# populationgenomics/cuKING

Measured on AMD Instinct MI355X. Metric: sample-pairs/s (all-pairs KING), higher is better.
Workload: dtype fp4 products, f32 accumulate (exact integers)

## Files before the change

cuking_amd/csrc/king_abi.hip:

```cpp
#include <hip/hip_runtime.h>

#include <algorithm>
#include <cstdio>
#include <cstdlib>
#include <cstring>
#include <vector>

#include "king_common.h"
#include "king_geno.h"
#include "king_host.h"
#include "king_ibd.h"
#include "king_kin_summary.h"
#include "king_ld.h"
#include "king_site_qc.h"
#include "king_unrelated.h"

using namespace cuking;

namespace {

#define HIP_TRY(expr)                                                      \
  do {                                                                     \
    const hipError_t _e = (expr);                                          \
    if (_e != hipSuccess) {                                                \
// ... 380 lines not shown
  a.result_index = out.result_index;
  a.result_overflow = out.result_overflow;
  a.dense_counts = out.counts;
  a.dense_kin = out.kin;
  a.kin_ld = out.kin_ld;
  a.kin_diag = (out.kin != nullptr && (out.kin_flags & CUKING_KIN_SYMMETRIC)) ? 1u : 0u;
  a.sum_hist = reinterpret_cast<unsigned long long *>(out.sum_hist);
  a.sum_best = reinterpret_cast<unsigned long long *>(out.sum_best);
  if (out.sum_hist != nullptr) {
    a.sum_lo = out.sum_bins.lo;
    a.sum_scale = kin_bin_scale(out.sum_bins);
    a.sum_bins = out.sum_bins.num_bins;
  }
  a.rel_counts = out.rel_counts;
  if (out.rel_counts != nullptr) {
    a.rel_num = out.rel_num;
    for (uint32_t t = 0; t < out.rel_num; ++t) a.rel_thr[t] = out.rel_thr[t];
  }
  a.rect_row_stride = 1;
  a.bits = d_bit_sets;
  a.words_per_sample = words_per_sample;
  a.split_wgs = ctx->split_wgs;
  if (plan_variant(ctx, words_per_sample).layout == kLayoutNibbleStats) {
    a.perm = plane_perm(ctx->planes, geo);
    if (!ctx->prepared.codes) a.codes_ready = plane_flags(ctx->planes, geo);
  }
  cuking_ctx::StreamScratch *e;
  const cuking_status st = scratch_for(ctx, stream, block_tiles, &e);
  if (st != CUKING_OK || e == nullptr) return st;
  if (uses_split_slab(ctx)) {
    a.split_counters = e->split;
    a.split_scratch = e->split + mfma_split_counter_bytes(ctx->split_wgs) / sizeof(uint32_t);
  }
  if (!uses_filter_scratch(ctx)) return CUKING_OK;
  uint8_t *base = e->filter;
  const FilterScratchLayout l = filter_scratch_layout(e->filter_tiles);
  a.sample_stats = plane_stats(ctx->planes, geo);
  a.t2 = plane_t2(ctx->planes, geo);
  a.prefix_u = plane_prefix_u(ctx->planes, geo);
  a.cohort_sums = plane_cohort_sums(ctx->planes, geo);
  a.filter_ctrl = reinterpret_cast<uint32_t *>(base);
  a.filter_totals = reinterpret_cast<unsigned long long *>(base + l.totals);
  a.fsplit_tickets = reinterpret_cast<uint32_t *>(base + l.tickets);
  a.tile_done = base + l.tile_done;
  a.cand_list = reinterpret_cast<uint2 *>(base + l.cand);
  a.cand_cap = ctx->filter_cand_cap < l.cand_entries ? ctx->filter_cand_cap : l.cand_entries;
  a.quadrant_cap = ctx->filter_quadrant_cap;
  a.dense_list = reinterpret_cast<uint2 *>(base + l.dense);
  a.dense_cap = l.chunk_tiles * 4;
  a.fsplit_slabs = ctx->split_wgs != 0 ? reinterpret_cast<float4 *>(base + l.slabs) : nullptr;
  a.rotate_min_steps = ctx->filter_rotate_min_steps;
  a.check_steps = plane_check_steps(ctx->planes, geo);
  if (ctx->prepared.site_order) a.site_curve = plane_site_curve(ctx->planes, geo);
  a.site_rotate = ctx->filter_site_order == 2;
  return CUKING_OK;
}

hipError_t launch_planned(const cuking_ctx *ctx, uint32_t words_per_sample, bool full,
                          TiledArgs a, const LaunchSwitches &sw, uint64_t num_tiles,
                          hipStream_t stream) {
  const int kv = effective_variant(ctx, words_per_sample);
  if (tiled_variant(kv).tile != tiled_variant(ctx->variant).tile) {
    if (tiled_variant(kv).tile * 2 != tiled_variant(ctx->variant).tile) return hipErrorInvalidValue;
    to_quadrants(&a, &num_tiles);
  }
  return launch_tiled(kv, full, a, sw, num_tiles, stream);
}

void note_reader(cuking_ctx *ctx, hipStream_t stream) {
  for (auto &r : ctx->readers)
    if (r.first == stream) return;
  ctx->readers.emplace_back(stream, nullptr);
}

cuking_status wait_for_readers(cuking_ctx *ctx, hipStream_t stream) {
  bool failed = false;
  for (auto &r : ctx->readers) {
    if (r.first == stream) continue;
    if (r.second == nullptr &&
        hipEventCreateWithFlags(&r.second, hipEventDisableTiming) != hipSuccess) {
      failed = true;
      break;
    }
    if (hipEventRecord(r.second, r.first) != hipSuccess ||
        hipStreamWaitEvent(stream, r.second, 0) != hipSuccess) {
      failed = true;
      break;
    }
  }
  if (failed) {
    (void)hipGetLastError();
    ++ctx->host_syncs;
    HIP_TRY(hipDeviceSynchronize());
  }
  for (auto &r : ctx->readers)
    if (r.second) (void)hipEventDestroy(r.second);
  ctx->readers.clear();
  ctx->readers.emplace_back(stream, nullptr);
  ctx->prepared.ordered_on = stream;
  ctx->prepared.ordered_valid = true;
  for (auto &t : ctx->prepared.tiles)
    if (t == 2) t = 1;
  return CUKING_OK;
}

void mark_read(cuking_ctx *ctx, uint32_t begin, uint32_t end) {
  std::vector<uint8_t> &t = ctx->prepared.tiles;
// ... 1693 lines not shown
```

cuking_amd/csrc/king_common.h:

```cpp
#ifndef CUKING_AMD_KING_COMMON_H_
#define CUKING_AMD_KING_COMMON_H_

#include <hip/hip_runtime.h>
#include <stdint.h>

#include "cuking_amd.h"
#include "king_launch_plan.h"
#include "king_submatrix.h"

namespace cuking {

constexpr uint32_t kLayoutWord = 0;
constexpr uint32_t kLayoutQuad = 1;
constexpr uint32_t kLayoutNibble = 2;
constexpr uint32_t kLayoutNibbleStats = 3;

struct PlaneGeometry {
  uint32_t num_rows, num_cols;
  uint32_t rows_padded, cols_padded;
  uint32_t col_base;
  uint32_t s_stride;
  uint32_t k_words;
  uint32_t diag;
};
// ... 50 lines not shown
  uint32_t i_begin, j_begin;
  float kin_threshold;
  uint32_t max_results;
  cuking_result *results;
  uint32_t *result_index;
  uint32_t *result_overflow;
  cuking_counts *dense_counts;
  const uint64_t *bits;
  uint32_t words_per_sample;
  uint32_t split_tiles, split_wgs;
  uint32_t split_whole;
  uint32_t *split_scratch, *split_counters;
  uint32_t xcd_chunk, launch_tiles;
  uint32_t dyn_tiles, dyn_wgs;
  uint32_t quad;
  const uint2 *tile_list;
  const uint32_t *tile_list_count;
  uint32_t tile_list_cap;
  const float2 *sample_stats;
  const uint4 *t2;
  uint32_t *filter_ctrl;
  unsigned long long *filter_totals;
  uint2 *cand_list;
  uint32_t cand_cap;
  uint32_t quadrant_cap;
  uint2 *dense_list;
  uint32_t dense_cap;
  uint32_t fsplit_parts, fsplit_first, fsplit_tile0;
  float4 *fsplit_slabs;
  uint32_t *fsplit_tickets;
  const uint32_t *check_steps;
  const float *prefix_u;
  const unsigned long long *cohort_sums;
  uint32_t check0, check1;
  uint32_t rotate, rotate_min_steps;
  uint32_t rotate_min_tiles;
  uint8_t *tile_done;
  const uint32_t *gate;
  uint32_t gate_count;
  const uint8_t *skip_tiles;
  uint64_t skip_base;
  const uint32_t *perm;
  uint32_t *codes_ready;
  float *dense_kin;
  uint64_t kin_ld;
  uint32_t kin_diag;
  unsigned long long *sum_hist, *sum_best;
  float sum_lo, sum_scale;
  uint32_t sum_bins;
  uint32_t *rel_counts;
  uint32_t rel_num;
  float rel_thr[CUKING_REL_THRESHOLDS_MAX];
  const struct SiteCurve *site_curve;
  uint32_t site_rotate;
};

constexpr uint32_t kCheckEmitCap = 64;
constexpr uint32_t kNumCheckShares = 8;
constexpr uint32_t kCheckShares64[kNumCheckShares] = {8, 50, 53, 56, 58, 60, 61, 62};
constexpr uint32_t kNumPhases = 128;
constexpr uint32_t kPhasesPerShare = kNumPhases / 64;
constexpr uint32_t kNumCum = kNumPhases - 1;
__host__ __device__ inline uint32_t phase_step(uint32_t all_steps, uint32_t x) {
  return (uint32_t)((uint64_t)all_steps * x / kNumPhases);
}
constexpr uint64_t kSiteOrderMinTiles = 24576;
constexpr uint32_t kSiteOrderMinGain = 2;
constexpr uint32_t kSiteOrderNoTrust = 15;
struct SiteCurve {
  unsigned long long cum[kNumPhases];
  unsigned long long het_calls, missing_calls;
  float sigma;
  uint32_t pad[11];
};
static_assert(sizeof(SiteCurve) % 64 == 0, "whole 64-byte lines");
__host__ __device__ inline float site_curve_mass(const unsigned long long *cum, uint32_t phase,
                                                 uint32_t share64) {
  const uint32_t hi = phase + share64 * kPhasesPerShare;
  auto front = [&](uint32_t x) { return x == 0 ? 0ull : cum[x - 1]; };
  const unsigned long long all = cum[kNumPhases - 1];
  const unsigned long long got = hi <= kNumPhases ? front(hi) - front(phase)
                                                  : (all - front(phase)) + front(hi - kNumPhases);
  return all != 0 ? (float)got / (float)all : 0.f;
}
__host__ __device__ inline bool site_curve_covers(const unsigned long long *cum, uint32_t phase,
                                                  uint32_t share64, float need) {
  return site_curve_mass(cum, phase, share64) >= need;
}
__host__ __device__ inline uint32_t check_step_of(uint32_t all_steps, uint32_t k,
                                                  uint32_t min_steps = 64) {
  if (all_steps < min_steps) return 0;
  return phase_step(all_steps, kCheckShares64[k] * kPhasesPerShare);
}
constexpr uint32_t kFilterSplitSlabs = 256;
constexpr size_t kFilterSlabBytes = 256 * 256 * sizeof(float);
constexpr size_t kFilterTicketBytes = kFilterSplitSlabs * sizeof(uint32_t);
__host__ __device__ inline size_t plane_bytes(const PlaneGeometry &g,
                                              uint32_t layout) {
  const size_t base = (size_t)g.k_words * g.s_stride * (layout == kLayoutQuad ? 8 : 16);
  if (layout == kLayoutNibble) return base + base / 4;
  if (layout == kLayoutNibbleStats)
    return base + base / 4 + base / 2 + (size_t)g.s_stride * sizeof(float2) +
           (size_t)g.s_stride * kNumCum * sizeof(float) + 64 + 64 +
           64 + (size_t)g.s_stride * (4 + 8 + 4 * (kNumCum + 1) + 16) +
           sizeof(SiteCurve);
  return base;
}
__host__ __device__ inline const uint4 *plane_t2(const uint4 *planes, const PlaneGeometry &g) {
  return planes + (size_t)g.k_words * g.s_stride * 5 / 4;
}
__host__ __device__ inline const float2 *plane_stats(const uint4 *planes, const PlaneGeometry &g) {
  return reinterpret_cast<const float2 *>(planes + (size_t)g.k_words * g.s_stride * 7 / 4);
}
__host__ __device__ inline const float *plane_prefix_u(const uint4 *planes, const PlaneGeometry &g) {
  return reinterpret_cast<const float *>(plane_stats(planes, g) + g.s_stride);
}
__host__ __device__ inline const unsigned long long *plane_cohort_sums(const uint4 *planes,
                                                                       const PlaneGeometry &g) {
  return reinterpret_cast<const unsigned long long *>(plane_prefix_u(planes, g) +
                                                      (size_t)g.s_stride * kNumCum);
}
// ... 266 lines not shown
```

cuking_amd/csrc/king_filter.hip:

```cpp
#include <hip/hip_runtime.h>
#include <stdio.h>

#include <atomic>
#include <stdlib.h>

#include "king_common.h"
#include "king_device.h"
#include "king_kin_summary.h"

#pragma clang diagnostic ignored "-Winline-asm"

namespace cuking {

namespace {

typedef int v8i __attribute__((ext_vector_type(8)));
typedef float v16f __attribute__((ext_vector_type(16)));

constexpr int kT = (int)kFilterTile;
constexpr int kUnits = 2;
constexpr int kStages = 5;
constexpr int kSliceU4 = kT;
constexpr int kStageU4 = 2 * 2 * kUnits * kSliceU4;
constexpr int kStageReqs = 4 * kUnits;
// ... 110 lines not shown
  r[1] = (int)(w.y & mask);
  r[2] = (int)(w.z & mask);
  r[3] = (int)(w.w & mask);
  return r;
}

struct Tile {
  bool split;
  uint32_t bid;
  uint32_t tr, tc;
  uint32_t part, piece;
};

__device__ __forceinline__ bool bound_level(const unsigned long long *cohort_sums, float sites,
                                            float *mean, float *sigma) {
  const float ns = (float)cohort_sums[0], nm = (float)cohort_sums[1], nh = (float)cohort_sums[2];
  if (!(ns > 0.f && nh > 0.f)) return false;
  const float m = nm / (ns * sites), h = nh / (ns * sites);
  *mean = m * (1.f + m / (2.f * h * (1.f - m)));
  *sigma = rsqrtf(sites);
  return true;
}

__device__ __forceinline__ bool take_tile(const TiledArgs &a, const uint32_t wg, uint4 *const lds,
                                          Tile *t) {
  uint32_t bid = wg;
  t->split = a.fsplit_parts != 0 && wg >= a.fsplit_first;
  t->part = t->piece = 0;
  if (t->split) {
    t->piece = wg - a.fsplit_first;
    t->part = __builtin_amdgcn_readfirstlane(t->piece % a.fsplit_parts);
    bid = a.fsplit_tile0 + t->piece / a.fsplit_parts;
  } else
  if (a.dyn_tiles != 0 && wg >= a.launch_tiles) {
    uint32_t *slot = reinterpret_cast<uint32_t *>(lds);
    if (threadIdx.x == 0) *slot = relaxed_add(a.filter_ctrl + kCtrlDyn, 1u);
    __syncthreads();
    const uint32_t next = __builtin_amdgcn_readfirstlane(*slot);
    __syncthreads();
    if (next >= a.dyn_tiles) return false;
    bid = a.launch_tiles + next;
  } else if (a.xcd_chunk == 1) {
    bid = xcd_patch_tile(bid);
    if (bid >= a.launch_tiles) return false;
  }
  t->bid = __builtin_amdgcn_readfirstlane(bid);
  uint32_t tr, tc;
  if (!decode_tile_space(a, a.tile_begin + t->bid, &tr, &tc)) return false;
  t->tr = __builtin_amdgcn_readfirstlane(tr);
  t->tc = __builtin_amdgcn_readfirstlane(tc);
  return true;
}

__device__ __forceinline__ uint32_t hook_phase(const TiledArgs &a, const Tile &t) {
  if (a.rotate < 2 || a.geo.k_words / 8 < a.rotate_min_steps) return 0;
  return (a.rotate == 2 ? t.bid * 37u + 11u : a.rotate - 3u) & (kNumPhases - 1);
}
__device__ __forceinline__ bool launch_verdict(const TiledArgs &a, const uint32_t wg,
                                               uint4 *const lds, uint32_t *xcd_pos,
                                               const uint32_t start_phase, uint32_t *order_share) {
  uint32_t *verdict = reinterpret_cast<uint32_t *>(lds);
  if (threadIdx.x == 0) {
    uint32_t leave = relaxed_load(a.filter_ctrl + kCtrlAllLeave);
    auto all_leave = [&] {
      leave = 1;
      relaxed_store(a.filter_ctrl + kCtrlAllLeave, 1u);
      relaxed_store(a.filter_ctrl + kCtrlGate, 1u);
    };
    float mean, sigma;
    if (leave == 0 && a.cohort_sums != nullptr && a.check_steps != nullptr &&
        bound_level(a.cohort_sums, 32.f * (float)a.geo.k_words, &mean, &sigma) &&
        mean - 4.f * sigma > a.kin_threshold && (a.check1 >> 16) != 0)
      all_leave();
    if (leave == 0) {
      const uint32_t dense_so_far =
          relaxed_load(a.filter_ctrl + kCtrlDense) + relaxed_load(a.filter_ctrl + kCtrlLeft);
      const uint32_t finished = relaxed_load(a.filter_ctrl + kCtrlFinished);
      if (finished >= 512 && 2 * dense_so_far > finished) all_leave();
    }
    verdict[0] = leave;
  }
  if (a.rotate == 1 && threadIdx.x < kPosSlots) {
    const uint32_t x = wg & 7;
    const unsigned long long said = relaxed_load(
        reinterpret_cast<const unsigned long long *>(a.filter_ctrl + kCtrlPos) + x * kPosSlots +
        threadIdx.x);
    const uint32_t ticks16 = relaxed_load(a.filter_ctrl + kCtrlStepTicks + x);
    uint32_t pos = (uint32_t)(said >> 32);
    const uint32_t ago = (uint32_t)__builtin_amdgcn_s_memrealtime() - (uint32_t)said;
    if (said != 0 && ticks16 != 0 && ago < 16384u)
      pos += ago * 16u / ticks16;
    verdict[1 + threadIdx.x] = pos;
  }
  if (a.site_curve != nullptr && (threadIdx.x >> 6) == 1) {
    const uint32_t s = threadIdx.x & 63;
    float mean, sigma;
    bool ok = false;
    if (a.cohort_sums != nullptr &&
        bound_level(a.cohort_sums, 32.f * (float)a.geo.k_words, &mean, &sigma)) {
      const float kappa = mean + 4.6f * a.site_curve->sigma + 0.003f;
      const float need = (1.f - 2.f * a.kin_threshold) / (1.f - 2.f * kappa);
      ok = kappa < 0.5f && s >= 32 && s <= 62 &&
           site_curve_covers(a.site_curve->cum, start_phase, s, need);
    }
    const unsigned long long fits = __ballot(ok);
    if (s == 0) verdict[1 + kPosSlots] = fits != 0 ? (uint32_t)__ffsll(fits) - 1u : 0u;
  }
  __syncthreads();
  *order_share = a.site_curve != nullptr ? __builtin_amdgcn_readfirstlane(verdict[1 + kPosSlots]) : 0u;
  const bool give_up = verdict[0] != 0;
  uint32_t pos = 0;
  if (a.rotate == 1) {
#pragma unroll
    for (uint32_t k = 0; k < kPosSlots; ++k) pos = max(pos, verdict[1 + k]);
  }
  *xcd_pos = __builtin_amdgcn_readfirstlane(pos);
  __syncthreads();
  if (give_up && threadIdx.x == 0) relaxed_add(a.filter_totals + kTotalDense, 4ull);
  return give_up;
}

struct CheckPlan {
  uint32_t chk0, chk1;
  uint32_t share1;
  uint32_t phase;
  uint32_t k0;
  uint32_t wrap;
  uint32_t start_abs;
};
__device__ __forceinline__ CheckPlan plan_checks(const TiledArgs &a, const Tile &t,
                                                 const uint32_t xcd_pos, const uint32_t order_share,
                                                 const uint32_t all_steps,
                                                 const uint32_t num_steps) {
  uint32_t chk0 = 0, chk1 = 0, entry1 = 0, share1 = 0;
  uint32_t phase = 0, k0 = 0, wrap = 0, start_abs = 0;
  if (!t.split && a.check_steps != nullptr && a.tile_done != nullptr) {
    if (a.rotate != 0 && all_steps >= a.rotate_min_steps) {
      uint32_t base = 0;
      if (a.rotate == 1) {
        const uint32_t r = xcd_pos % all_steps;
        base = xcd_pos - r;
        phase = (r * kNumPhases + all_steps / 2) / all_steps;
        if (phase >= kNumPhases) {
          phase = 0;
          base += all_steps;
        }
      } else if (a.rotate == 2) {
        phase = (t.bid * 37u + 11u) & (kNumPhases - 1);
      } else {
        phase = (a.rotate - 3u) & (kNumPhases - 1);
      }
      k0 = phase_step(all_steps, phase);
      start_abs = base + k0;
      wrap = k0 != 0 ? all_steps - k0 : 0u;
    }
    uint32_t curve_share = order_share;
    if (a.site_curve != nullptr && a.rotate == 1 && phase != 0) {
      curve_share = 0;
      float m0, s0;
      if (a.cohort_sums != nullptr && bound_level(a.cohort_sums, 256.f * (float)all_steps, &m0, &s0)) {
        const float kap = m0 + 4.6f * a.site_curve->sigma + 0.003f;
        const float need = (1.f - 2.f * a.kin_threshold) / (1.f - 2.f * kap);
        if (kap < 0.5f && site_curve_covers(a.site_curve->cum, phase, 62, need)) {
          uint32_t lo = 32, hi = 62;
          while (lo < hi) {
            const uint32_t mid = (lo + hi) / 2;
            if (site_curve_covers(a.site_curve->cum, phase, mid, need)) hi = mid;
            else lo = mid + 1;
          }
          curve_share = lo;
        }
      }
    }
    float kappa = -1.f, mean, sigma;
    if (bound_level(a.cohort_sums, 256.f * (float)all_steps, &mean, &sigma))
      kappa = mean + 4.6f * sigma + 0.003f;
    auto steps_of = [&](uint32_t share) {
      const uint32_t hi = phase + share * kPhasesPerShare;
      return hi <= kNumPhases ? phase_step(all_steps, hi) - k0
                              : (all_steps - k0) + phase_step(all_steps, hi - kNumPhases);
    };
    if ((a.check0 == 2 || (a.check0 == 1 && kappa > 0.7f * a.kin_threshold)) &&
        a.check_steps[0] != 0)
      chk0 = steps_of(kCheckShares64[0]);
    const uint32_t sw1 = a.check1 & 0xFFu;
    if (sw1 >= 2) {
      entry1 = sw1 - 2;
    } else if (sw1 == 1 && a.site_curve != nullptr) {
      if (curve_share != 0) {
        share1 = curve_share;
        entry1 = 1;
      }
    } else if (sw1 == 1 && kappa >= 0.f) {
      const float f64 = 64.f * (1.f - 2.f * a.kin_threshold) / (1.f - 2.f * kappa);
      if (f64 <= 62.f) {
        share1 = (uint32_t)ceilf(f64);
        if (share1 < 32) share1 = 32;
        entry1 = 1;
      }
    }
#pragma unroll
    for (uint32_t k = 1; k < kNumCheckShares; ++k)
      if (sw1 >= 2 && k == entry1) share1 = kCheckShares64[k];
    if (share1 != 0 && a.check_steps[entry1] != 0) chk1 = steps_of(share1);
    if (chk0 >= num_steps) chk0 = 0;
    if (chk1 >= num_steps || chk1 <= chk0) chk1 = 0;
  }
  auto sgpr = [](uint32_t v) { return (uint32_t)__builtin_amdgcn_readfirstlane(v); };
  return CheckPlan{sgpr(chk0), sgpr(chk1), sgpr(share1), sgpr(phase), sgpr(k0), sgpr(wrap), sgpr(start_abs)};
}

__device__ __forceinline__ float prefix_u_of(const TiledArgs &a, const CheckPlan &p,
                                             uint32_t share, size_t idx, float total) {
  const uint32_t s_stride = a.geo.s_stride;
  const uint32_t hi = p.phase + share * kPhasesPerShare;
  float u = hi >= kNumPhases ? total
            : hi != 0        ? a.prefix_u[(size_t)(hi - 1) * s_stride + idx]
                             : 0.f;
  if (p.phase != 0) u -= a.prefix_u[(size_t)(p.phase - 1) * s_stride + idx];
  if (hi > kNumPhases) u += a.prefix_u[(size_t)(hi - kNumPhases - 1) * s_stride + idx];
  return u;
}

__device__ __forceinline__ const float2 *stage_bounds(const TiledArgs &a, const Tile &t,
                                                      const CheckPlan &p, uint4 *const lds,
                                                      const bool prefix, const uint32_t share,
                                                      const float thr, const float scale) {
  float2 *const rows = reinterpret_cast<float2 *>(lds), *const cols = rows + kT;
  const float tt = 2.f - 4.f * thr;
  const size_t ir = (size_t)t.tr * kT + threadIdx.x;
  const size_t ic = (size_t)a.geo.col_base + (size_t)t.tc * kT + threadIdx.x;
  float2 r = a.sample_stats[ir], c = a.sample_stats[ic];
  if (prefix) {
    r.x = prefix_u_of(a, p, share, ir, r.x);
    c.x = prefix_u_of(a, p, share, ic, c.x);
  }
  r.y = scale * fmaf(tt, r.y, 8.f);
  c.y = scale * fmaf(tt, c.y, 8.f);
  rows[threadIdx.x] = r;
  cols[threadIdx.x] = c;
  __syncthreads();
  return rows;
}

enum Leave : uint32_t { kStays = 0, kLeftForecast, kLeftEmpty, kLeftEmit };

__device__ __forceinline__ Leave check_sweep(const TiledArgs &a, const Tile &t, const CheckPlan &p,
                                             const v16f (&acc)[4][4], uint4 *const lds,
                                             const bool forecast, const uint32_t all_steps) {
  const Lanes l = lanes_of_thread();
  const float scale = !forecast ? 1.f
                      : a.site_curve != nullptr
                          ? site_curve_mass(a.site_curve->cum, p.phase, kCheckShares64[0])
                          : (float)kCheckShares64[0] * (1.f / 64.f);
  const uint32_t share = forecast ? kCheckShares64[0] : p.share1;
  const float thr_f = forecast ? a.kin_threshold + 3.66f * rsqrtf(256.f * (float)all_steps)
                               : a.kin_threshold;
  const float2 *const ck_rows = stage_bounds(a, t, p, lds, true, share, thr_f, scale);
  const float2 *const ck_cols = ck_rows + kT;
  uint32_t *const ck_words = reinterpret_cast<uint32_t *>(lds) + 4 * kT;
  const uint32_t emit_cap = (a.check1 >> 8) & 0xFFu;
  uint32_t cnt = 0;
  {
    float2 cc[4];
#pragma unroll
    for (int bj = 0; bj < 4; ++bj) cc[bj] = ck_cols[l.wx * 128 + bj * 32 + l.lr];
#pragma unroll
    for (int bi = 0; bi < 4; ++bi)
#pragma unroll
      for (int r = 0; r < 16; ++r) {
        const float2 cr = ck_rows[l.wy * 128 + bi * 32 + c_row(r, l.g)];
#pragma unroll
        for (int bj = 0; bj < 4; ++bj)
          cnt += fmaf(-8.f, acc[bi][bj][r], cr.x) + cc[bj].x < fminf(cr.y, cc[bj].y) ? 1u : 0u;
      }
  }
#pragma unroll
  for (int off = 32; off > 0; off >>= 1) cnt += __shfl_xor(cnt, off);
  if (l.lane == 0)
    ck_words[l.wave] = forecast ? (cnt > 2 * a.quadrant_cap ? 1u : 0u)
                                : (cnt > emit_cap ? emit_cap + 1 : cnt);
  __syncthreads();
  uint32_t found = forecast ? ck_words[0] + ck_words[1] + ck_words[2] + ck_words[3]
                            : max(max(ck_words[0], ck_words[1]), max(ck_words[2], ck_words[3]));
  found = __builtin_amdgcn_readfirstlane(found);
  __syncthreads();
  if (forecast) return found >= 3 ? kLeftForecast : kStays;
  return found > emit_cap ? kStays : found != 0 ? kLeftEmit : kLeftEmpty;
}

__device__ __forceinline__ bool leave_early(const TiledArgs &a, const Tile &t, const CheckPlan &p,
                                            const Leave left) {
  if (left == kLeftEmit && threadIdx.x == 0) relaxed_add(a.filter_totals + kTotalEarly, 1ull);
  if (p.phase != 0 && threadIdx.x == 0) relaxed_add(a.filter_totals + kTotalRotated, 1ull);
  if (left == kLeftForecast || left == kLeftEmpty) {
    if (threadIdx.x == 0) {
      relaxed_add(a.filter_ctrl + kCtrlFinished, 4u);
      if (left == kLeftForecast) {
        relaxed_add(a.filter_ctrl + kCtrlLeft, 4u);
        relaxed_store(a.filter_ctrl + kCtrlGate, 1u);
        relaxed_add(a.filter_totals + kTotalDense, 4ull);
      } else {
        a.tile_done[t.bid] = 1;
        relaxed_add(a.filter_totals + kTotalEarly, 1ull);
      }
    }
// ... 203 lines not shown
    F_MMA(CUR, 1, 0) F_BAR                                                     \
    F_BUILD_A(NXT, 2) F_MMA(CUR, 1, 1) F_BAR                                   \
    F_MMA(CUR, 1, 2) F_BAR                                                     \
    F_BUILD_A(NXT, 3) F_MMA(CUR, 1, 3) F_BAR                                   \
    F_ISSUE(src_, dst_, OFF1);                                                 \
    F_MMA(CUR, 2, 0) F_BAR                                                     \
    F_BUILD_A(NXT, 4) F_MMA(CUR, 2, 1) F_BAR                                   \
    F_MMA(CUR, 2, 2) F_BAR                                                     \
    F_BUILD_A(NXT, 5) F_MMA(CUR, 2, 3) F_BAR                                   \
    F_MMA(CUR, 3, 0) F_BAR                                                     \
    F_BUILD_A(NXT, 6) F_MMA(CUR, 3, 1) F_BAR                                   \
    F_MMA(CUR, 3, 2) F_BAR                                                     \
    F_BUILD_A(NXT, 7) F_MMA(CUR, 3, 3) F_BAR                                   \
  }
#define F_SLICE_A(CUR, NXT, RBUF, RC, SYNC, PA, DC, OFF0, OFF1)                \
  {                                                                            \
    if (SYNC) {                                                                \
      __builtin_amdgcn_s_waitcnt(vmcnt_imm(kSyncVm));                          \
      __syncthreads();                                                         \
    }                                                                          \
    const char *src_ = (PA).src + (DC) * row_bytes;                            \
    const uint32_t dst_ = (PA).dst + (DC) * (kSliceU4 * 16);                   \
    F_READ(0, RBUF, RC) F_READ(1, RBUF, RC)                                    \
    F_ISSUE(src_, dst_, OFF0);                                                 \
    F_MMA(CUR, 0, 0) F_MMA(CUR, 0, 1) F_BAR                                    \
    F_READ(2, RBUF, RC) F_READ(3, RBUF, RC)                                    \
    F_MMA(CUR, 0, 2) F_MMA(CUR, 0, 3) F_BAR                                    \
    F_READ(4, RBUF, RC) F_READ(5, RBUF, RC)                                    \
    F_ISSUE(src_, dst_, OFF1);                                                 \
    F_MMA(CUR, 1, 0) F_MMA(CUR, 1, 1) F_BAR                                    \
    F_READ(6, RBUF, RC) F_READ(7, RBUF, RC)                                    \
    F_MMA(CUR, 1, 2) F_MMA(CUR, 1, 3) F_BAR                                    \
    F_BUILD_B(NXT, 0) F_MMA(CUR, 2, 0) F_BAR                                   \
    F_BUILD_B(NXT, 1) F_MMA(CUR, 2, 1) F_BAR                                   \
    F_BUILD_B(NXT, 2) F_MMA(CUR, 2, 2) F_BAR                                   \
    F_BUILD_B(NXT, 3) F_MMA(CUR, 2, 3) F_BAR                                   \
    F_BUILD_B(NXT, 4) F_MMA(CUR, 3, 0) F_BAR                                   \
    F_BUILD_B(NXT, 5) F_MMA(CUR, 3, 1) F_BAR                                   \
    F_BUILD_B(NXT, 6) F_MMA(CUR, 3, 2) F_BAR                                   \
    F_BUILD_B(NXT, 7) F_MMA(CUR, 3, 3) F_BAR                                   \
  }
#define F_KSTEP                                                                \
  {                                                                            \
    const uint32_t nbuf = buf == kStages - 1 ? 0 : buf + 1;                    \
    F_SLICE_B(0, 1, pa, 0, 0, 1024)                                            \
    F_SLICE_A(1, 0, buf, 1, false, pa, 0, 2048, 3072)                          \
    F_SLICE_B(0, 1, pa, 1, 0, 1024)                                            \
    F_SLICE_A(1, 0, nbuf, 0, true, pa, 1, 2048, 3072)                          \
    pa = addr_next(pa, step + kStages, buf);                                   \
    buf = nbuf;                                                                \
    ++step;                                                                    \
  }
#define F_PUBLISH(STEPS)                                                       \
  if (a.rotate == 1 && wave == 0) {                                            \
    const uint32_t now_ = (uint32_t)__builtin_amdgcn_s_memrealtime();          \
    const unsigned long long val_ =                                            \
        ((unsigned long long)(start_abs + (STEPS)) << 32) | now_;              \
     \
    const uint32_t t16_ = (STEPS) >= 32 ? (now_ - t_start) * 16u / (STEPS) : 0u; \
    const uint32_t zero_ = 0;                                                  \
    unsigned long long save_;                                                  \
    asm volatile("s_mov_b64 %0, exec\n\t"                                      \
                 "s_mov_b64 exec, 1\n\t"                                       \
                 "global_store_dwordx2 %1, %2, %3\n\t"                         \
                 "s_mov_b64 exec, %0"                                          \
                 : "=&s"(save_)                                                \
                 : "v"(zero_), "v"(val_), "s"(pos_word)                        \
                 : "memory");                                                  \
    if (t16_ != 0)                                                             \
      asm volatile("s_mov_b64 %0, exec\n\t"                                    \
                   "s_mov_b64 exec, 1\n\t"                                     \
                   "global_store_dword %1, %2, %3\n\t"                         \
                   "s_mov_b64 exec, %0"                                        \
                   : "=&s"(save_)                                              \
                   : "v"(zero_), "v"(t16_), "s"(ticks_word)                    \
                   : "memory");                                                \
  }

__device__ __forceinline__ void filter_tile(const TiledArgs &a, const uint32_t wg, uint4 *const lds) {
  Tile tile;
  if (!take_tile(a, wg, lds, &tile)) return;
  const Lanes ln = lanes_of_thread();
  uint32_t xcd_pos = 0, order_share = 0;
  if (!tile.split && a.tile_done != nullptr &&
      launch_verdict(a, wg, lds, &xcd_pos, hook_phase(a, tile), &order_share))
    return;
  const uint32_t all_steps = a.geo.k_words / (4 * kUnits);
  const uint32_t k_first = __builtin_amdgcn_readfirstlane(
      tile.split ? tile.part * all_steps / a.fsplit_parts : 0u);
  const uint32_t num_steps = __builtin_amdgcn_readfirstlane(
      tile.split ? (tile.part + 1) * all_steps / a.fsplit_parts - k_first : all_steps);
  const CheckPlan plan = plan_checks(a, tile, xcd_pos, order_share, all_steps, num_steps);

  const uint32_t wave = ln.wave, chk0 = plan.chk0, chk1 = plan.chk1;
  const uint32_t k0 = plan.k0, wrap = plan.wrap, start_abs = plan.start_abs;
  uint32_t lane16 = ln.lane * 16;
  const uint32_t s_stride = a.geo.s_stride;
  const uint4 *g_rows = a.t2 + (uint64_t)tile.tr * kT;
  const uint4 *g_cols = a.t2 + a.geo.col_base + (uint64_t)tile.tc * kT;

  uint32_t mT, mA;
  asm volatile("s_mov_b32 %0, 0xcccccccc" : "=s"(mT));
  asm volatile("s_mov_b32 %0, 0x33333333" : "=s"(mA));
  int scaleB;
  asm volatile("v_mov_b32 %0, 0x7d7d7d7d" : "=v"(scaleB));

  const uint32_t dma_side = wave >> 1, dma_h = wave & 1;
  const uint32_t row_bytes = s_stride * 16;
  const char *const g_wave = reinterpret_cast<const char *>(
      (dma_side ? g_cols : g_rows) + ((uint64_t)2 * kUnits * k_first + kUnits * dma_h) * s_stride);
  const uint32_t l_wave = (uint32_t)(uintptr_t)(lds_void_ptr)(
      lds + ((dma_side * 2 + dma_h) * kUnits) * kSliceU4);
  struct Addr { const char *src; uint32_t dst; };
  const uint32_t kstep_bytes = 2 * kUnits * row_bytes;
  const char *seg_src = g_wave;
  uint32_t seg_steps = num_steps;
  uint32_t seg_wrap = 0xFFFFFFFFu;
  auto addr_of = [&](uint32_t step, uint32_t buf) {
    Addr pa;
    if (step >= seg_steps) step = seg_steps - 1;
    const int32_t rel = (int32_t)step - (int32_t)(step >= seg_wrap ? all_steps : 0u);
    pa.src = seg_src + (int64_t)rel * (int64_t)kstep_bytes;
    pa.dst = l_wave + buf * (kStageU4 * 16);
    asm volatile("" : "+s"(pa.src), "+s"(pa.dst));
    return pa;
  };
  auto addr_next = [&](const Addr &cur, uint32_t step, uint32_t buf) {
    Addr pa;
    const int32_t adv = (int32_t)(step < seg_steps ? 1u : 0u) -
                        (int32_t)(step == seg_wrap ? all_steps : 0u);
    pa.src = cur.src + (int64_t)adv * (int64_t)kstep_bytes;
    pa.dst = l_wave + buf * (kStageU4 * 16);
    asm volatile("" : "+s"(pa.src), "+s"(pa.dst));
    return pa;
  };

  v16f acc[4][4] = {};

  uint32_t row_off = ((0 * 2 + ln.g) * kUnits) * kSliceU4 + ln.wy * 128 + ln.lr;
  uint32_t col_off = ((1 * 2 + ln.g) * kUnits) * kSliceU4 + ln.wx * 128 + ln.lr;
  asm volatile("" : "+v"(row_off), "+v"(col_off), "+v"(lane16));
  v8i FA[2][4], FB[2][4];
  uint4 RAW[8];

  unsigned long long *const pos_word =
      reinterpret_cast<unsigned long long *>(a.filter_ctrl + kCtrlPos) +
      (wg & 7) * kPosSlots + ((wg >> 3) & (kPosSlots - 1));
  uint32_t *const ticks_word = a.filter_ctrl + kCtrlStepTicks + (wg & 7);
  const uint32_t t_start = a.rotate == 1 ? (uint32_t)__builtin_amdgcn_s_memrealtime() : 0u;

  uint32_t seg_first = 0;
  Leave left = kStays;
#pragma nounroll
  while (true) {
    uint32_t seg_end = num_steps;
    if (chk1 > seg_first) seg_end = chk1;
    if (chk0 > seg_first) seg_end = chk0;
    seg_end = __builtin_amdgcn_readfirstlane(seg_end);
    seg_steps = seg_end - seg_first;
    const uint32_t seg_k = seg_first >= wrap && wrap != 0 ? seg_first - wrap : k0 + seg_first;
    seg_src = g_wave + (uint64_t)seg_k * kstep_bytes;
    seg_wrap = __builtin_amdgcn_readfirstlane(
        wrap > seg_first && wrap < seg_end ? wrap - seg_first : 0xFFFFFFFFu);
    asm volatile("" : "+s"(seg_src), "+s"(seg_steps), "+s"(seg_wrap));

#pragma unroll
    for (int st = 0; st < kStages - 1; ++st) {
      const Addr p0 = addr_of(st, st);
      F_ISSUE4(p0, 0)
      F_ISSUE4(p0, 1)
    }
    __builtin_amdgcn_s_waitcnt(vmcnt_imm((kStages - 2) * kStageReqs));
    __syncthreads();
#pragma unroll
    for (int k = 0; k < 8; ++k) {
      F_READ(k, 0, 0)
    }
#pragma unroll
    for (int k = 0; k < 8; ++k) {
      F_BUILD_B(0, k)
    }
    uint32_t buf = 0;
    Addr pa = addr_of(kStages - 1, kStages - 1);
    uint32_t step = 0;
    while (step + 1 < seg_steps) {
      F_KSTEP
      F_KSTEP
    }
    if (step < seg_steps) F_KSTEP
    __builtin_amdgcn_s_waitcnt(0x0F70);
    __syncthreads();
    F_PUBLISH(seg_end)
    if (seg_end == num_steps) break;

    left = check_sweep(a, tile, plan, acc, lds, seg_end == chk0, all_steps);
    if (left != kStays) break;
    seg_first = seg_end;
  }

  if (leave_early(a, tile, plan, left)) return;
  if (tile.split && !reduce_pieces(a, tile, acc, lds)) return;
  emit_candidates(a, tile, plan, acc, lds, left == kLeftEmit);
}
#undef F_KSTEP
#undef F_SLICE_A
#undef F_SLICE_B
#undef F_BAR
#undef F_MMA
#undef F_BUILD_A
#undef F_BUILD_B
#undef F_PIN4
#undef F_PINF
#undef F_READ
// ... 116 lines not shown
      s_opp += __shfl_xor(s_opp, off);
    }
    if (lane == 0) {
      const uint32_t band = rel_band(a.rel_thr, a.rel_num, king_kinship(s_het_i, s_het_j, s_both, s_opp));
      if (band != kRelNoBand) {
        atomicAdd(a.rel_counts + (size_t)off_i * a.rel_num + band, 1u);
        atomicAdd(a.rel_counts + (size_t)off_j * a.rel_num + band, 1u);
      }
    }
  }
}

}

static std::atomic<uint32_t> g_check_min_steps{64};
void set_filter_check_min_steps(uint32_t steps) { g_check_min_steps.store(steps); }
uint32_t filter_check_min_steps() { return g_check_min_steps.load(); }

hipError_t launch_sample_stats(const uint64_t *d_bit_sets, uint32_t words_per_sample,
                               const PlaneGeometry &geo, uint4 *d_planes, uint32_t s_begin,
                               uint32_t s_end, hipStream_t stream) {
  if (s_end > geo.s_stride) s_end = geo.s_stride;
  if (s_begin >= s_end) return hipSuccess;
  float2 *stats = plane_tmp_stats(d_planes, geo);
  float *prefix = plane_tmp_prefix(d_planes, geo);
  unsigned long long *sums = const_cast<unsigned long long *>(plane_cohort_sums(d_planes, geo));
  uint32_t *steps = const_cast<uint32_t *>(plane_check_steps(d_planes, geo));
  CheckWords cw;
  const uint32_t all_steps = geo.k_words / 8;
  if (all_steps > kStatsMaxSteps) return hipErrorInvalidValue;
  for (uint32_t k = 0; k < kNumCheckShares; ++k)
    cw.w[k] = check_step_of(all_steps, k, g_check_min_steps.load());
  sample_stats_kernel<<<dim3((s_end - s_begin + 3) / 4), dim3(256), 0, stream>>>(
      d_bit_sets, words_per_sample, geo, stats, prefix, sums, steps, cw, s_begin, s_end);
  return hipGetLastError();
}

hipError_t launch_filter(const TiledArgs &args, const LaunchSwitches &switches, uint64_t num_tiles,
                         hipStream_t stream) {
  if ((uint64_t)args.geo.k_words * 32 > kMfmaN4MaxSites || args.filter_ctrl == nullptr ||
      args.cand_list == nullptr || args.dense_list == nullptr || args.sample_stats == nullptr)
    return hipErrorInvalidValue;
  if (args.rel_counts != nullptr && (args.rel_num == 0 || args.rel_num > CUKING_REL_THRESHOLDS_MAX))
    return hipErrorInvalidValue;
  hipError_t e = allow_dynamic_lds<king_filter_kernel>(kFilterLdsBytes);
  if (e != hipSuccess) return e;
  uint64_t cap = max_blocks_per_launch(256);
  if (cap > kFilterChunkTiles) cap = kFilterChunkTiles;
  if (cap > args.dense_cap / 4) cap = args.dense_cap / 4;
  if (cap == 0) return hipErrorInvalidValue;
  const uint32_t wgs = args.split_wgs != 0 ? args.split_wgs : 256;
  const bool checks = args.tile_done != nullptr;
  LaunchSwitches sw = switches;
  if (args.site_curve != nullptr && sw.rotate == 1 && args.site_rotate == 0) sw.rotate = 0;
  const bool can_split = args.fsplit_slabs != nullptr && args.fsplit_tickets != nullptr;
  for (uint64_t done = 0; done < num_tiles;) {
    const FilterPlan p = filter_plan(num_tiles - done, cap, wgs, args.geo.k_words / 8, checks,
                                     can_split, kFilterSplitSlabs, sw);
    e = hipMemsetAsync(args.filter_ctrl, 0, kCtrlChunkBytes + (checks ? p.n : 0), stream);
    if (e != hipSuccess) return e;
    TiledArgs chunk = args;
    chunk.tile_begin = args.tile_begin + done;
    TiledArgs a = chunk;
    a.check0 = p.check0;
    a.check1 = p.check1;
    a.rotate = p.rotate;
    a.launch_tiles = p.whole.launch_tiles;
    a.xcd_chunk = p.whole.xcd_chunk;
    a.dyn_tiles = p.whole.dyn_tiles;
    a.dyn_wgs = p.whole.dyn_wgs;
    a.fsplit_parts = p.parts;
    a.fsplit_tile0 = p.fsplit_tile0;
    a.fsplit_first = p.fsplit_first;
    if (checks && p.rest != 0) {
      e = hipMemsetAsync(args.tile_done + p.fsplit_tile0, 1, p.rest, stream);
      if (e != hipSuccess) return e;
    }
    king_filter_kernel<<<dim3((uint32_t)p.grid), dim3(256), kFilterLdsBytes, stream>>>(a);
    e = hipGetLastError();
    if (e != hipSuccess) return e;
    if (a.rel_counts != nullptr) king_refine_count_kernel<<<dim3(wgs * 4), dim3(256), 0, stream>>>(a);
    else king_refine_kernel<<<dim3(wgs * 4), dim3(256), 0, stream>>>(a);
    e = hipGetLastError();
    if (e != hipSuccess) return e;
    if (a.codes_ready != nullptr) {
      e = launch_prepare_nibbles(true, false, a.bits, a.words_per_sample, a.geo,
                                 const_cast<uint4 *>(a.planes), a.perm, 0, 0xFFFFFFFFu,
                                 a.filter_ctrl, a.codes_ready, stream);
      if (e != hipSuccess) return e;
      e = launch_mark_codes_ready(a.filter_ctrl, a.codes_ready, stream);
      if (e != hipSuccess) return e;
    }
    e = launch_mfma_list(chunk, args.dense_list, args.filter_ctrl + kCtrlDense, args.dense_cap,
                         wgs, stream);
    if (e != hipSuccess) return e;
    if (checks) {
      TiledArgs f = chunk;
      uint64_t units = p.n;
      to_quadrants(&f, &units);
      e = launch_mfma_gated(f, units, args.filter_ctrl + kCtrlGate, args.tile_done,
                            chunk.tile_begin, wgs, stream);
      if (e != hipSuccess) return e;
    }
    done += p.n;
  }
  return hipSuccess;
}
// ... 3 lines not shown
```

Before: 41.52 billion.

## Rotate filter start within the site-ordered head ring instead of full K

When a site-ordered curve is present, the filter kernel now rotates each tile's start phase only within the head of the k range that the order-share check covers (a 'ring'), so the early-exit check at the ring's end sees the high-information sites regardless of rotation. The old per-phase curve-share search and hook_phase are removed, and prefix counts use a separate count phase. Auto site order now enables this lap mode by default. This aims to keep the DRAM/L2 load spread from rotation while preserving the early-termination savings of site ordering, at the cost of more complex segment/wrap addressing.

```diff
diff --git a/cuking_amd/csrc/king_abi.hip b/cuking_amd/csrc/king_abi.hip
--- a/cuking_amd/csrc/king_abi.hip
+++ b/cuking_amd/csrc/king_abi.hip
@@ -456,7 +456,7 @@
   a.rotate_min_steps = ctx->filter_rotate_min_steps;
   a.check_steps = plane_check_steps(ctx->planes, geo);
   if (ctx->prepared.site_order) a.site_curve = plane_site_curve(ctx->planes, geo);
-  a.site_rotate = ctx->filter_site_order == 2;
+  a.site_lap = ctx->filter_site_order == 2 || (ctx->filter_site_order == -1 && kSiteOrderAutoLap);
   return CUKING_OK;
 }
 
diff --git a/cuking_amd/csrc/king_common.h b/cuking_amd/csrc/king_common.h
--- a/cuking_amd/csrc/king_common.h
+++ b/cuking_amd/csrc/king_common.h
@@ -126,7 +126,7 @@
   uint32_t rel_num;
   float rel_thr[CUKING_REL_THRESHOLDS_MAX];
   const struct SiteCurve *site_curve;
-  uint32_t site_rotate;
+  uint32_t site_lap;
 };
 
 constexpr uint32_t kCheckEmitCap = 64;
@@ -141,6 +141,7 @@
 constexpr uint64_t kSiteOrderMinTiles = 24576;
 constexpr uint32_t kSiteOrderMinGain = 2;
 constexpr uint32_t kSiteOrderNoTrust = 15;
+constexpr bool kSiteOrderAutoLap = true;
 struct SiteCurve {
   unsigned long long cum[kNumPhases];
   unsigned long long het_calls, missing_calls;
diff --git a/cuking_amd/csrc/king_filter.hip b/cuking_amd/csrc/king_filter.hip
--- a/cuking_amd/csrc/king_filter.hip
+++ b/cuking_amd/csrc/king_filter.hip
@@ -186,13 +186,9 @@
   return true;
 }
 
-__device__ __forceinline__ uint32_t hook_phase(const TiledArgs &a, const Tile &t) {
-  if (a.rotate < 2 || a.geo.k_words / 8 < a.rotate_min_steps) return 0;
-  return (a.rotate == 2 ? t.bid * 37u + 11u : a.rotate - 3u) & (kNumPhases - 1);
-}
 __device__ __forceinline__ bool launch_verdict(const TiledArgs &a, const uint32_t wg,
                                                uint4 *const lds, uint32_t *xcd_pos,
-                                               const uint32_t start_phase, uint32_t *order_share) {
+                                               uint32_t *order_share) {
   uint32_t *verdict = reinterpret_cast<uint32_t *>(lds);
   if (threadIdx.x == 0) {
     uint32_t leave = relaxed_load(a.filter_ctrl + kCtrlAllLeave);
@@ -235,7 +231,7 @@
       const float kappa = mean + 4.6f * a.site_curve->sigma + 0.003f;
       const float need = (1.f - 2.f * a.kin_threshold) / (1.f - 2.f * kappa);
       ok = kappa < 0.5f && s >= 32 && s <= 62 &&
-           site_curve_covers(a.site_curve->cum, start_phase, s, need);
+           site_curve_covers(a.site_curve->cum, 0, s, need);
     }
     const unsigned long long fits = __ballot(ok);
     if (s == 0) verdict[1 + kPosSlots] = fits != 0 ? (uint32_t)__ffsll(fits) - 1u : 0u;
@@ -260,6 +256,8 @@
   uint32_t phase;
   uint32_t k0;
   uint32_t wrap;
+  uint32_t ring;
+  uint32_t count_phase;
   uint32_t start_abs;
 };
 __device__ __forceinline__ CheckPlan plan_checks(const TiledArgs &a, const Tile &t,
@@ -267,62 +265,52 @@
                                                  const uint32_t all_steps,
                                                  const uint32_t num_steps) {
   uint32_t chk0 = 0, chk1 = 0, entry1 = 0, share1 = 0;
-  uint32_t phase = 0, k0 = 0, wrap = 0, start_abs = 0;
+  uint32_t phase = 0, k0 = 0, wrap = 0, start_abs = 0, ring = all_steps;
+  bool lap = false;
   if (!t.split && a.check_steps != nullptr && a.tile_done != nullptr) {
-    if (a.rotate != 0 && all_steps >= a.rotate_min_steps) {
-      uint32_t base = 0;
-      if (a.rotate == 1) {
-        const uint32_t r = xcd_pos % all_steps;
-        base = xcd_pos - r;
-        phase = (r * kNumPhases + all_steps / 2) / all_steps;
-        if (phase >= kNumPhases) {
-          phase = 0;
-          base += all_steps;
-        }
-      } else if (a.rotate == 2) {
-        phase = (t.bid * 37u + 11u) & (kNumPhases - 1);
-      } else {
-        phase = (a.rotate - 3u) & (kNumPhases - 1);
-      }
-      k0 = phase_step(all_steps, phase);
-      start_abs = base + k0;
-      wrap = k0 != 0 ? all_steps - k0 : 0u;
-    }
-    uint32_t curve_share = order_share;
-    if (a.site_curve != nullptr && a.rotate == 1 && phase != 0) {
-      curve_share = 0;
-      float m0, s0;
-      if (a.cohort_sums != nullptr && bound_level(a.cohort_sums, 256.f * (float)all_steps, &m0, &s0)) {
-        const float kap = m0 + 4.6f * a.site_curve->sigma + 0.003f;
-        const float need = (1.f - 2.f * a.kin_threshold) / (1.f - 2.f * kap);
-        if (kap < 0.5f && site_curve_covers(a.site_curve->cum, phase, 62, need)) {
-          uint32_t lo = 32, hi = 62;
-          while (lo < hi) {
-            const uint32_t mid = (lo + hi) / 2;
-            if (site_curve_covers(a.site_curve->cum, phase, mid, need)) hi = mid;
-            else lo = mid + 1;
-          }
-          curve_share = lo;
-        }
-      }
-    }
     float kappa = -1.f, mean, sigma;
     if (bound_level(a.cohort_sums, 256.f * (float)all_steps, &mean, &sigma))
       kappa = mean + 4.6f * sigma + 0.003f;
+    const bool take0 = (a.check0 == 2 || (a.check0 == 1 && kappa > 0.7f * a.kin_threshold)) &&
+                       a.check_steps[0] != 0;
+    const uint32_t sw1 = a.check1 & 0xFFu;
+    const uint32_t head = order_share * kPhasesPerShare;
+    const uint32_t k_head = phase_step(all_steps, head);
+    lap = a.site_curve != nullptr && a.rotate != 0 && order_share != 0 && sw1 == 1 && !take0 &&
+          a.check_steps[1] != 0 && k_head >= a.rotate_min_steps && k_head < num_steps;
+    if (lap) ring = k_head;
+    const uint32_t ring_phases = lap ? head : kNumPhases;
+    if (a.rotate != 0 && (lap || (a.site_curve == nullptr && all_steps >= a.rotate_min_steps))) {
+      uint32_t base = 0;
+      if (a.rotate == 1) {
+        const uint32_t r = xcd_pos % ring;
+        base = xcd_pos - r;
+        phase = (r * kNumPhases + all_steps / 2) / all_steps;
+      } else if (a.rotate == 2) {
+        phase = ((t.bid * 37u + 11u) & (kNumPhases - 1)) % ring_phases;
+      } else {
+        phase = ((a.rotate - 3u) & (kNumPhases - 1)) % ring_phases;
+      }
+      k0 = phase_step(all_steps, phase);
+      if (phase >= ring_phases || k0 >= ring) {
+        phase = 0;
+        k0 = 0;
+        base += ring;
+      }
+      start_abs = base + k0;
+      wrap = k0 != 0 ? ring - k0 : 0u;
+    }
     auto steps_of = [&](uint32_t share) {
       const uint32_t hi = phase + share * kPhasesPerShare;
       return hi <= kNumPhases ? phase_step(all_steps, hi) - k0
                               : (all_steps - k0) + phase_step(all_steps, hi - kNumPhases);
     };
-    if ((a.check0 == 2 || (a.check0 == 1 && kappa > 0.7f * a.kin_threshold)) &&
-        a.check_steps[0] != 0)
-      chk0 = steps_of(kCheckShares64[0]);
-    const uint32_t sw1 = a.check1 & 0xFFu;
+    if (take0) chk0 = steps_of(kCheckShares64[0]);
     if (sw1 >= 2) {
       entry1 = sw1 - 2;
     } else if (sw1 == 1 && a.site_curve != nullptr) {
-      if (curve_share != 0) {
-        share1 = curve_share;
+      if (order_share != 0) {
+        share1 = order_share;
         entry1 = 1;
       }
     } else if (sw1 == 1 && kappa >= 0.f) {
@@ -336,22 +324,24 @@
 #pragma unroll
     for (uint32_t k = 1; k < kNumCheckShares; ++k)
       if (sw1 >= 2 && k == entry1) share1 = kCheckShares64[k];
-    if (share1 != 0 && a.check_steps[entry1] != 0) chk1 = steps_of(share1);
+    if (share1 != 0 && a.check_steps[entry1] != 0) chk1 = lap ? ring : steps_of(share1);
     if (chk0 >= num_steps) chk0 = 0;
     if (chk1 >= num_steps || chk1 <= chk0) chk1 = 0;
   }
   auto sgpr = [](uint32_t v) { return (uint32_t)__builtin_amdgcn_readfirstlane(v); };
-  return CheckPlan{sgpr(chk0), sgpr(chk1), sgpr(share1), sgpr(phase), sgpr(k0), sgpr(wrap), sgpr(start_abs)};
+  return CheckPlan{sgpr(chk0), sgpr(chk1), sgpr(share1), sgpr(phase), sgpr(k0),
+                   sgpr(wrap), sgpr(ring), sgpr(lap ? 0u : phase), sgpr(start_abs)};
 }
 
 __device__ __forceinline__ float prefix_u_of(const TiledArgs &a, const CheckPlan &p,
                                              uint32_t share, size_t idx, float total) {
   const uint32_t s_stride = a.geo.s_stride;
-  const uint32_t hi = p.phase + share * kPhasesPerShare;
+  const uint32_t from = p.count_phase;
+  const uint32_t hi = from + share * kPhasesPerShare;
   float u = hi >= kNumPhases ? total
             : hi != 0        ? a.prefix_u[(size_t)(hi - 1) * s_stride + idx]
                              : 0.f;
-  if (p.phase != 0) u -= a.prefix_u[(size_t)(p.phase - 1) * s_stride + idx];
+  if (from != 0) u -= a.prefix_u[(size_t)(from - 1) * s_stride + idx];
   if (hi > kNumPhases) u += a.prefix_u[(size_t)(hi - kNumPhases - 1) * s_stride + idx];
   return u;
 }
@@ -385,7 +375,7 @@
   const Lanes l = lanes_of_thread();
   const float scale = !forecast ? 1.f
                       : a.site_curve != nullptr
-                          ? site_curve_mass(a.site_curve->cum, p.phase, kCheckShares64[0])
+                          ? site_curve_mass(a.site_curve->cum, p.count_phase, kCheckShares64[0])
                           : (float)kCheckShares64[0] * (1.f / 64.f);
   const uint32_t share = forecast ? kCheckShares64[0] : p.share1;
   const float thr_f = forecast ? a.kin_threshold + 3.66f * rsqrtf(256.f * (float)all_steps)
@@ -695,12 +685,12 @@
     ++step;                                                                    \
   }
 #define F_PUBLISH(STEPS)                                                       \
-  if (a.rotate == 1 && wave == 0) {                                            \
+  if (a.rotate == 1 && wave == 0 && (STEPS) <= ring) {                         \
     const uint32_t now_ = (uint32_t)__builtin_amdgcn_s_memrealtime();          \
     const unsigned long long val_ =                                            \
         ((unsigned long long)(start_abs + (STEPS)) << 32) | now_;              \
-     \
-    const uint32_t t16_ = (STEPS) >= 32 ? (now_ - t_start) * 16u / (STEPS) : 0u; \
+        \
+    const uint32_t t16_ = (STEPS) >= 16 ? (now_ - t_start) * 16u / (STEPS) : 0u; \
     const uint32_t zero_ = 0;                                                  \
     unsigned long long save_;                                                  \
     asm volatile("s_mov_b64 %0, exec\n\t"                                      \
@@ -726,7 +716,7 @@
   const Lanes ln = lanes_of_thread();
   uint32_t xcd_pos = 0, order_share = 0;
   if (!tile.split && a.tile_done != nullptr &&
-      launch_verdict(a, wg, lds, &xcd_pos, hook_phase(a, tile), &order_share))
+      launch_verdict(a, wg, lds, &xcd_pos, &order_share))
     return;
   const uint32_t all_steps = a.geo.k_words / (4 * kUnits);
   const uint32_t k_first = __builtin_amdgcn_readfirstlane(
@@ -736,7 +726,7 @@
   const CheckPlan plan = plan_checks(a, tile, xcd_pos, order_share, all_steps, num_steps);
 
   const uint32_t wave = ln.wave, chk0 = plan.chk0, chk1 = plan.chk1;
-  const uint32_t k0 = plan.k0, wrap = plan.wrap, start_abs = plan.start_abs;
+  const uint32_t k0 = plan.k0, wrap = plan.wrap, ring = plan.ring, start_abs = plan.start_abs;
   uint32_t lane16 = ln.lane * 16;
   const uint32_t s_stride = a.geo.s_stride;
   const uint4 *g_rows = a.t2 + (uint64_t)tile.tr * kT;
@@ -762,7 +752,7 @@
   auto addr_of = [&](uint32_t step, uint32_t buf) {
     Addr pa;
     if (step >= seg_steps) step = seg_steps - 1;
-    const int32_t rel = (int32_t)step - (int32_t)(step >= seg_wrap ? all_steps : 0u);
+    const int32_t rel = (int32_t)step - (int32_t)(step >= seg_wrap ? ring : 0u);
     pa.src = seg_src + (int64_t)rel * (int64_t)kstep_bytes;
     pa.dst = l_wave + buf * (kStageU4 * 16);
     asm volatile("" : "+s"(pa.src), "+s"(pa.dst));
@@ -771,7 +761,7 @@
   auto addr_next = [&](const Addr &cur, uint32_t step, uint32_t buf) {
     Addr pa;
     const int32_t adv = (int32_t)(step < seg_steps ? 1u : 0u) -
-                        (int32_t)(step == seg_wrap ? all_steps : 0u);
+                        (int32_t)(step == seg_wrap ? ring : 0u);
     pa.src = cur.src + (int64_t)adv * (int64_t)kstep_bytes;
     pa.dst = l_wave + buf * (kStageU4 * 16);
     asm volatile("" : "+s"(pa.src), "+s"(pa.dst));
@@ -801,7 +791,9 @@
     if (chk0 > seg_first) seg_end = chk0;
     seg_end = __builtin_amdgcn_readfirstlane(seg_end);
     seg_steps = seg_end - seg_first;
-    const uint32_t seg_k = seg_first >= wrap && wrap != 0 ? seg_first - wrap : k0 + seg_first;
+    const uint32_t seg_k = seg_first >= ring                ? seg_first
+                           : seg_first >= wrap && wrap != 0 ? seg_first - wrap
+                                                            : k0 + seg_first;
     seg_src = g_wave + (uint64_t)seg_k * kstep_bytes;
     seg_wrap = __builtin_amdgcn_readfirstlane(
         wrap > seg_first && wrap < seg_end ? wrap - seg_first : 0xFFFFFFFFu);
@@ -1024,7 +1016,7 @@
   const uint32_t wgs = args.split_wgs != 0 ? args.split_wgs : 256;
   const bool checks = args.tile_done != nullptr;
   LaunchSwitches sw = switches;
-  if (args.site_curve != nullptr && sw.rotate == 1 && args.site_rotate == 0) sw.rotate = 0;
+  if (args.site_curve != nullptr && sw.rotate == 1 && args.site_lap == 0) sw.rotate = 0;
   const bool can_split = args.fsplit_slabs != nullptr && args.fsplit_tickets != nullptr;
   for (uint64_t done = 0; done < num_tiles;) {
     const FilterPlan p = filter_plan(num_tiles - done, cap, wgs, args.geo.k_words / 8, checks,
```

Result: faster. 43.11 billion, median of 6 (+3.8%).
